# CookiePPP/cookietts

Hardware: AMD Instinct MI355X
Metric: audio samples/sec (22.05kHz) WaveGlow infer, 80×900 mel, 1/2/4/8 GPU; real-time factor (higher is better)
Workload: dtype f32; 1 GPU; WaveGlow full (12 flows, 512 WN ch, 8 groups, 8 layers) fp32 infer, batch 8 x (80x900) mel per GPU, sigma 0.6, random-init weights; batch_per_gpu=8, frames=900, parallelism=utterance-batch shard x1

## Files before the change

### cookietts_amd/_lib.py

```python
from __future__ import annotations

import ctypes as C
import os
import threading

import torch

from . import build as _build

_LOCK = threading.Lock()
_LIB = None


class WaveGlowConfig(C.Structure):
    _fields_ = [(n, C.c_int32) for n in (
        "n_mel_channels", "n_group", "n_flows", "n_early_every", "n_early_size",
        "win_length", "hop_length", "n_layers", "n_channels", "kernel_size", "cond_hidden", "speaker_embed_dim",
        "f32_gemm_mode")]


class StftConfig(C.Structure):
    _fields_ = [("filter_length", C.c_int32), ("hop_length", C.c_int32), ("win_length", C.c_int32),
                ("n_mel_channels", C.c_int32), ("clamp_val", C.c_float)]

# ... 269 lines not shown
                                           C.c_size_t, _FP]),
    "ctts_hifigan_packed_bf16x3_bytes": (C.c_size_t, [C.POINTER(HifiganConfig)]),
    "ctts_hifigan_pack_bf16x3": (C.c_int, [C.POINTER(HifiganConfig), _FP, C.c_size_t, _FP, _FP]),
    "ctts_hifigan_workspace_bf16x3_bytes": (C.c_size_t, [C.POINTER(HifiganConfig), C.c_int32, C.c_int32]),
    "ctts_hifigan_forward_bf16x3": (C.c_int, [C.POINTER(HifiganConfig), _FP, _FP, C.c_int32, _FP, C.c_int32, C.c_int32, _FP,
                                              C.c_size_t, _FP]),
    "ctts_replicate_halo_f32":(C.c_int, [_FP, C.c_int32, C.c_int32, C.c_int32, C.c_int32, C.c_int32, C.c_int32, _FP]),
    "ctts_embed_rows_f32": (C.c_int, [_FP, _FP, _FP, C.c_int32, C.c_int32, C.c_int32, C.c_int32, C.c_int32, C.c_int32,
                                      C.c_int32, _FP]),
    "ctts_scale_add_rows_f32": (C.c_int, [_FP, _FP, _FP, _FP, C.c_int32, C.c_int32, C.c_int32, C.c_int32, C.c_int32,
                                          _FP]),
    "ctts_deemphasis_f32": (C.c_int, [_FP, _FP, C.c_int32, C.c_int32, C.c_double, _FP]),
    "ctts_alignment_workspace_bytes": (C.c_size_t, [C.c_int32, C.c_int32, C.c_int32]),
    "ctts_alignment_metric_f32": (C.c_int, [_FP, _FP, _FP, C.c_int32, C.c_int32, C.c_int32, C.c_float, _FP, _FP,
                                            C.c_size_t, _FP]),
    "ctts_first_over_thresh_f32": (C.c_int, [_FP, C.c_int32, C.c_int32, C.c_float, _FP, _FP]),
    "ctts_taco_stop_state_bytes": (C.c_size_t, [C.c_int32]),
    "ctts_taco_stop_reset": (C.c_int, [_FP, C.c_int32, C.c_int32, _FP]),
    "ctts_taco_stop_rule_f32": (C.c_int, [_FP, C.c_int32, C.c_int32, C.c_int32, C.c_int32, C.c_float, C.c_int32, _FP, _FP]),
    "ctts_retry_state_bytes": (C.c_size_t, [C.POINTER(RetryConfig)]),
    "ctts_retry_state_layout": (C.c_int, [C.POINTER(RetryConfig), C.POINTER(C.c_size_t)]),
    "ctts_retry_reset": (C.c_int, [C.POINTER(RetryConfig), _FP, _FP]),
    "ctts_retry_update_f32": (C.c_int, [C.POINTER(RetryConfig), _FP, _FP, _FP, _FP, _FP, _FP, C.c_int32, C.c_int32, _FP, _FP,
                                        _FP]),
    "ctts_retry_vocoder_batch_f32": (C.c_int, [C.POINTER(RetryConfig), _FP, _FP, C.c_int32, C.c_float, _FP]),
    "ctts_pcm16_concat": (C.c_int, [_FP, C.c_int32, _FP, C.c_int32, C.c_int64, C.c_int32, C.c_int32, _FP, C.c_int64, _FP,
                                    _FP]),
    "ctts_affine_rows_f32": (C.c_int, [_FP, C.c_int32, C.c_int32, C.c_int32, C.c_int32, C.c_int32, C.c_int32, C.c_float,
                                       C.c_float, _FP]),
    "ctts_vol_unscale_f32": (C.c_int, [_FP, C.c_int64, _FP]),
    "ctts_resample_rows_f32": (C.c_int, [_FP, _FP] + [C.c_int32] * 9 + [C.c_float, _FP]),
    "ctts_interleave_phases_f32": (C.c_int, [_FP, _FP] + [C.c_int32] * 10 + [_FP]),
    "ctts_last_gemm_loop": (C.c_int, []),
    "ctts_tuning_reload": (C.c_int, []),
    "ctts_tuning_flags": (C.c_int, []),
    "ctts_profile_create": (C.c_int, [C.POINTER(C.c_void_p)]),
    "ctts_profile_bind": (C.c_int, [C.c_void_p]),
    "ctts_profile_collect": (C.c_int, [C.c_void_p, C.c_int32, C.POINTER(C.c_int64), C.POINTER(C.c_double)]),
    "ctts_profile_destroy": (C.c_int, [C.c_void_p]),
}

MODEL_GEMM_MODES = {None: 0, "default": 0, "f32": 1, "bf16x3": 2, "bf16x6": 3}
GEMM_MODES = {"f32": 1, "bf16x3": 2, "bf16x6": 3}


def model_gemm_mode(mode):
    try:
        return MODEL_GEMM_MODES[mode]
    except KeyError:
        raise ValueError(f"f32 GEMM mode {mode!r}: expected one of 'default', 'f32', 'bf16x3', 'bf16x6'") from None


def set_f32_gemm_mode(mode):
    if mode in (None, "default", "f32"):
        return "f32"
    raise RuntimeError(f"cookietts_amd.set_f32_gemm_mode({mode!r}): the process-wide default was removed; "
                       f"call model.set_f32_gemm_mode({mode!r}) on each model instead")


class Profile:

    def __init__(self):
        h = C.c_void_p()
        check(lib().ctts_profile_create(C.byref(h)), "ctts_profile_create")
        self._h = h

# ... 121 lines not shown
```

### cookietts_amd/csrc/waveglow_api.hip

```cpp
#include <mutex>
#include <vector>

#include "gemm_bf16.h"
#include "gemm_f32.h"
#include "tuning.h"
#include "waveglow_kernels.h"
#include "wn_winograd_layer.h"

namespace ctts {

static thread_local char g_err[512] = "";

void set_error(const char* fmt, ...) {
    va_list ap;
    va_start(ap, fmt);
    vsnprintf(g_err, sizeof(g_err), fmt, ap);
    va_end(ap);
}

namespace {

constexpr size_t ALIGN_F = 64;
inline size_t align_up(size_t v) { return (v + ALIGN_F - 1) / ALIGN_F * ALIGN_F; }
constexpr int A_TILE = GEMM_KC * GEMM_BM;
// ... 121 lines not shown

struct Geom { int L, ld, pad, ntiles; };

int make_geom(const Plan& p, int frames, Geom& g) {
    CTTS_CHECK_ARG(frames >= 1, "frames=%d", frames);
    const long long T = (long long)frames * p.c.hop_length;
    g.L = (int)(T / p.c.n_group);
    int maxd = 1 << (p.c.n_layers - 1);
    g.pad = round_up(maxd > 128 ? maxd : 128, 32);
    g.ntiles = (g.L + GEMM_BN - 1) / GEMM_BN;
    g.ld = round_up(g.L, 256) + 2 * g.pad;
    return CTTS_OK;
}

struct PairGeom { int d, Lp, ntiles; };
PairGeom pair_geom(const Geom& g, int layer) {
    const int d = 1 << layer;
    const int Lp = (g.L + 2 * d - 1) / (2 * d) * d;
    return {d, Lp, (Lp + GEMM_BN - 1) / GEMM_BN};
}
int pair_ld(const Plan& p, const Geom& g) {
    int nt = 0;
    for (int i = 0; i < p.c.n_layers; ++i) nt = std::max(nt, pair_geom(g, i).ntiles);
    return nt * GEMM_BN;
}
PairGeom quad_geom(const Geom& g, int layer) {
    const int d = 1 << layer;
    const int Lq = (g.L + 4 * d - 1) / (4 * d) * d;
    return {d, Lq, (Lq + 63) / 64};
}
int quad_ld(const Plan& p, const Geom& g) {
    int nt = 0;
    for (int i = 0; i < p.c.n_layers; ++i) nt = std::max(nt, quad_geom(g, i).ntiles);
    return nt * 64;
}
constexpr long long WINOGRAD_MIN_COLS = 28800;
bool winograd_engages(const Plan& p, const Geom& g) {
    const Tuning t = tuning();
    if (t.f32_no_winograd || gemm_split_level(p.c.f32_gemm_mode) != 0) return false;
    const long long min_cols = t.f32_winograd_min >= 0 ? t.f32_winograd_min : WINOGRAD_MIN_COLS;
    return (long long)g.L >= min_cols;
}

constexpr long long WINOGRAD_FUSED_MIN_COLS = 28800;
bool winograd_fused_engages(const Plan& p, const Geom& g) {
    const Tuning t = tuning();
    if (t.f32_winograd_no_fused || t.f32_winograd_plain || t.f32_no_glds || !wn_winograd_layer_supported(p.C, p.H)) return false;
    const long long min_cols = t.f32_winograd_fused_min >= 0 ? t.f32_winograd_fused_min : WINOGRAD_FUSED_MIN_COLS;
    return winograd_engages(p, g) && (long long)g.L >= min_cols;
}

constexpr long long WINOGRAD_F43_MIN_COLS = 28800;
bool winograd_f43_engages(const Plan& p, const Geom& g) {
    const Tuning t = tuning();
    if (t.f32_winograd_no_f43 || !wn_winograd_layer_f43_supported(p.C, p.H) || !gemm_f32_dma_staged(p.nch_rs + p.nch1h)) return false;
    const long long min_cols = t.f32_winograd_f43_min >= 0 ? t.f32_winograd_f43_min : WINOGRAD_F43_MIN_COLS;
    return winograd_fused_engages(p, g) && (long long)g.L >= min_cols;
}

struct Workspace {
    float *audio, *spect, *spk, *h_tmp, *h_all, *x, *act, *out;
    float* act_all;
    float* a16;
    float* skend;
    float *wgV, *wgT, *wgH;
    int ldp, ldq;
    size_t total;
// ... 96 lines not shown
        a.nseg = 2;
        a.seg[1] = {spk, (long long)p.c.n_flows * p.S * g.ld, p.S / GEMM_KC, 0, p.S, 0};
    }
    a.dst0 = h_tmp; a.dst0_bstride = hstride; a.acc0 = 0;
    a.dst1 = h_tmp; a.dst1_bstride = hstride; a.acc1 = 0;
    a.split = p.c.n_flows * GEMM_BM;
    a.M = p.c.n_flows * GEMM_BM;
    int rc = launch_gemm_f32(GEMM_EPI_SPLIT, a, s);
    if (rc) return rc;
    a.A = blob + p.cond1_A; a.bias = blob + p.cond1_b;
    a.nseg = 1; a.nch_total = p.nch1h;
    a.seg[0] = {h_tmp, hstride, p.nch1h, 0, GEMM_BM, 0};
    a.dst0 = h_all; a.dst1 = h_all;
    return launch_gemm_f32(GEMM_EPI_SPLIT, a, s);
}

struct WnFold { float* a16; float* skend; float* audio; float* wave; };
struct WnWinograd { float* V; float* T; float* Hc; int ldp; int ldq; };

int run_in_layer_winograd(const Plan& p, const Geom& g, const float* blob, int k, int i, const float* x, const float* h_all,
                          float* act, const WnWinograd& wg, int batch, hipStream_t s) {
    const auto& f = p.fl[k];
    const PairGeom pg = pair_geom(g, i);
    const int C = p.C, H = p.H, ldp = wg.ldp;
    const long long hstride = (long long)p.c.n_flows * H * g.ld;
    const size_t vplane = (size_t)batch * C * ldp, tplane = (size_t)batch * 2 * C * ldp, hplane = (size_t)batch * H * ldp;
    const bool lean = !tuning().f32_winograd_plain && gemm_f32_dma_staged(p.nch_rs + p.nch1h);
    const bool in_place = lean && pg.d % 4 == 0;
    const bool fused = lean && winograd_fused_engages(p, g);
    const float* h2 = h_all + (size_t)k * H * g.ld;
    if (fused && wg.ldq > 0 && winograd_f43_engages(p, g)) {
        const PairGeom qg = quad_geom(g, i);
        const int ldq = wg.ldq;
        int rc = launch_winograd_transform_quad(x, (long long)C * g.ld, h2, hstride, wg.V, wg.Hc, batch, C, H, qg.d, g.L, qg.Lp, g.ld, g.pad,
                                                ldq, qg.ntiles * 64, !in_place, s);
        if (rc) return rc;
        WnWinogradLayerArgs w{};
        w.form = WNWG_F43;
        w.A_T2 = blob + f.wq_U_A[0][i]; w.A_T3 = blob + f.wq_U_A[1][i]; w.A_T4 = blob + f.wq_U_A[2][i]; w.A_T5 = blob + f.wq_U_A[3][i];
        w.A_e = blob + f.wq_e_A[i]; w.A_o = blob + f.wq_o_A[i];
        w.bias = blob + f.in_b[i];
        w.V = wg.V; w.vplane = (long long)batch * C * ldq;
        w.Hc = wg.Hc; w.hplane = (long long)batch * H * ldq;
        w.h2 = h2; w.h_bstride = hstride;
        w.act = act; w.act_bstride = (long long)C * g.ld;
        w.C = C; w.H = H; w.batch = batch;
        w.ldp = ldq; w.Lp = qg.Lp; w.ntiles = qg.ntiles;
        w.d = qg.d; w.L = g.L; w.ld = g.ld; w.pad = g.pad;
        w.in_place = in_place;
        return launch_wn_winograd_layer(w, s);
    }
    int rc = launch_winograd_transform(x, (long long)C * g.ld, h2, hstride, wg.V, wg.Hc, batch, C, H, pg.d, g.L, pg.Lp, g.ld, g.pad,
                                       ldp, pg.ntiles * GEMM_BN, !in_place, lean, s);
    if (rc) return rc;
    if (fused) {
        WnWinogradLayerArgs w{};
        w.A_T2 = blob + f.wg_T2_A[i]; w.A_T3 = blob + f.wg_T3_A[i]; w.A_e = blob + f.wg_e_A[i]; w.A_o = blob + f.wg_o_A[i];
        w.bias = blob + f.in_b[i];
        w.V = wg.V; w.vplane = (long long)vplane;
        w.Hc = wg.Hc; w.hplane = (long long)hplane;
        w.h2 = h2; w.h_bstride = hstride;
        w.act = act; w.act_bstride = (long long)C * g.ld;
        w.C = C; w.H = H; w.batch = batch;
        w.ldp = ldp; w.Lp = pg.Lp; w.ntiles = pg.ntiles;
        w.d = pg.d; w.L = g.L; w.ld = g.ld; w.pad = g.pad;
        w.in_place = in_place;
        return launch_wn_winograd_layer(w, s);
    }
// ... 806 lines not shown
}

int ctts_waveglow_infer_spk_f32(const ctts_waveglow_config* cfg, const void* packed, const float* mel,
                                const float* z_scaled, const int64_t* speaker_ids, float* wave, int32_t batch,
                                int32_t frames, void* workspace, size_t workspace_bytes, void* stream) {
    Plan p; Geom g; Workspace w;
    int rc = make_plan(cfg, p); if (rc) return rc;
    rc = make_geom(p, frames, g); if (rc) return rc;
    CTTS_CHECK_ARG(packed && mel && z_scaled && wave && workspace && batch >= 1, "infer: bad argument");
    carve(p, g, batch, static_cast<float*>(workspace), w);
    if (w.total * sizeof(float) > workspace_bytes) {
        set_error("infer: workspace %zu bytes < required %zu", workspace_bytes, w.total * sizeof(float));
        return CTTS_E_WORKSPACE;
    }
    hipStream_t s = as_stream(stream);
    const float* blob = static_cast<const float*>(packed);
    CTTS_CHECK_HIP(hipMemcpyAsync(w.audio, z_scaled, (size_t)batch * p.c.n_group * g.L * sizeof(float),
                                  hipMemcpyDeviceToDevice, s));
    rc = launch_upsample_squeeze(mel, blob + p.up_w, p.up_mfma ? blob + p.up_wp : nullptr, blob + p.up_b, w.spect, batch, p.c.n_mel_channels, frames,
                                 p.c.win_length, p.c.hop_length, p.c.n_group, g.ld, g.pad, s);
    if (rc) return rc;
    rc = fill_speaker_rows(p, g, blob, speaker_ids, w.spk, batch, s);
    if (rc) return rc;
    rc = run_cond(p, g, blob, w.spect, w.spk, w.h_tmp, w.h_all, batch, s);
    if (rc) return rc;
    for (int k = p.c.n_flows - 1; k >= 0; --k) {
        rc = run_flow(p, g, blob, k, w, w.audio, w.h_all, k == 0 ? wave : nullptr, batch, s);
        if (rc) return rc;
    }
    return CTTS_OK;
}

int ctts_last_gemm_loop(void) { return last_gemm_loop(); }
int ctts_tuning_reload(void) { reload_tuning(); return CTTS_OK; }
int ctts_tuning_flags(void) {
    const Tuning t = tuning();
    return (t.f32_no_glds ? 1 : 0) | (t.no_xcd_pair ? 2 : 0) | (t.bf16_no_wide ? 8 : 0) | (t.bf16_no_pp ? 16 : 0) |
           (t.wf_no_fuse ? 128 : 0) | (t.taco_no_fuse ? 256 : 0) | (t.f32_no_small ? 512 : 0) | (t.f32_force_small ? 1024 : 0) |
           (t.f32_no_splitk ? 2048 : 0) | (t.wf_no_vec_interp ? 4096 : 0) | (t.f32_no_defer_skip ? 8192 : 0) |
           (t.wf_no_region_split ? 16384 : 0) | (t.wf_no_row_queue ? 32768 : 0) | (t.wf_row_queue_min >= 0 ? 65536 : 0) |
           (t.wf_inject_abort ? 131072 : 0) | (t.wf_queue_debug ? 262144 : 0) | (t.f32_no_round_split ? 524288 : 0) |
           (t.bf16_ps ? (1 << 20) : 0) | (t.bf16_no_ps ? (1 << 21) : 0) | (t.taco_poll_delay_set ? (1 << 23) : 0) |
           (t.taco_valu ? (1 << 24) : 0) | (t.up_no_mfma ? (1 << 25) : 0) | (t.f32_no_wn_fold ? (1 << 26) : 0) |
           (t.taco_bg_no_pipe ? (1 << 27) : 0) | (t.f32_no_winograd ? (1 << 28) : 0) | (t.f32_winograd_min >= 0 ? (1 << 29) : 0) |
           (t.f32_winograd_plain ? (1 << 30) : 0) | (t.f32_winograd_fused_min >= 0 ? 4 : 0) | (t.f32_winograd_no_fused ? 32 : 0) |
           (t.f32_winograd_f43_min >= 0 ? (1 << 6) : 0) | (t.f32_winograd_no_f43 ? (1 << 22) : 0) |
           (t.wf_fwd_rowwise ? (int)(1u << 31) : 0);
}

int ctts_profile_create(void** handle) {
    CTTS_CHECK_ARG(handle, "profile_create: NULL");
    *handle = new Prof();
    return CTTS_OK;
}

int ctts_profile_bind(void* handle) {
    t_prof = static_cast<Prof*>(handle);
    return CTTS_OK;
}

int ctts_profile_collect(void* handle, int32_t which, int64_t* launches, double* total_ms) {
    Prof* pr = static_cast<Prof*>(handle);
    CTTS_CHECK_ARG(pr && which >= 0 && which < CTTS_PROF_N && launches && total_ms, "profile_collect: bad argument");
    std::lock_guard<std::mutex> lk(pr->mu);
    double tot = 0.0;
    int64_t n = 0;
// ... 218 lines not shown
```

### cookietts_amd/csrc/wn_winograd_layer.h

```cpp
#pragma once

#include "common.h"
#include "gemm_f32.h"

namespace ctts {

constexpr int WNWG_MAX_CHUNKS = 320;
constexpr int WNWG_F23 = 0, WNWG_F43 = 1;

struct WnWinogradLayerArgs {
    const float *A_T2, *A_T3, *A_e, *A_o, *bias;
    const float *A_T4, *A_T5;
    const float* V; long long vplane;
    const float* Hc; long long hplane;
    const float* h2; long long h_bstride;
    float* act; long long act_bstride;
    int C, H, batch;
    int ldp, Lp, ntiles;
    int d, L, ld, pad;
    int in_place;
    int form;
    int kt, kt_total, b0, col0;
};

bool wn_winograd_layer_supported(int C, int H);
bool wn_winograd_layer_f43_supported(int C, int H);
int launch_wn_winograd_layer(const WnWinogradLayerArgs& a, hipStream_t stream);

}
```

### cookietts_amd/csrc/wn_winograd_layer.hip

```cpp
#include "wn_winograd_layer.h"
#include "tuning.h"

namespace ctts {

typedef float wg_f32x16 __attribute__((ext_vector_type(16)));

namespace {

__device__ __forceinline__ float wg_sigmoid(float u) {
    return __builtin_amdgcn_rcpf(1.0f + __builtin_amdgcn_exp2f(u * -1.4426950408889634f));
}
__device__ __forceinline__ float wg_tanh(float u) {
    return 1.0f - 2.0f * __builtin_amdgcn_rcpf(1.0f + __builtin_amdgcn_exp2f(u * 2.8853900817779268f));
}

}

template <int NT, int F43>
__global__ __launch_bounds__(256, 2) void wn_winograd_layer_f32_kernel(const WnWinogradLayerArgs a) {
    static_assert(!F43 || NT == 1, "the F(4,3) form runs on the 64-column shape");
    constexpr int NI = F43 ? 4 : 2;
    constexpr int BN = 64 * NT;
    constexpr int A_ST = GEMM_KC * 128;
    constexpr int STG = A_ST + GEMM_KC * BN;
    constexpr int TAB = 3 * STG;
    constexpr int BIAS = TAB + 4 * WNWG_MAX_CHUNKS;
    constexpr int UPR = BN / 4;
    constexpr int RPP = 64 / UPR;
    __shared__ __attribute__((aligned(16))) float lds[BIAS + 128];

    const int t = threadIdx.x;
    const int lane = t & 63;
    const int wave = __builtin_amdgcn_readfirstlane(t >> 6);
    const int wm = wave >> 1, wn = wave & 1;
    const int l31 = lane & 31, lhi = lane >> 5;

    const int ncb = a.C >> 6;
    const int jx = blockIdx.x >> 3;
    const int cb = jx % ncb;
    const int gt = (jx / ncb) * 8 + (blockIdx.x & 7);
    if (gt >= a.kt_total) return;
    const int b = a.b0 + gt / a.kt;
    const int n0 = a.col0 + (gt % a.kt) * BN;

    const int n1 = a.C / GEMM_KC, n2 = (a.C + a.H) / GEMM_KC, nh = a.H / GEMM_KC;
    const int c_e = NI * n1;
    int ps[NI + 1];
    ps[0] = c_e;
#pragma unroll
    for (int k = 0; k < NI; ++k) ps[k + 1] = ps[k] + (k == 0 || k == NI - 1 ? n2 : nh);
    const int nch = ps[NI];

    const int mb_t = (64 * cb) >> 8, loc_t = (64 * cb) & 255;
    const int mb_s = (a.C + 64 * cb) >> 8, loc_s = (a.C + 64 * cb) & 255;
    {
        uint4* tab = reinterpret_cast<uint4*>(lds + TAB);
        for (int c = t; c < nch; c += 256) {
// ... 33 lines not shown
#pragma unroll
        for (int j = 0; j < NT; ++j) {
            const int krow = (wave + 4 * j) * RPP + lane / UPR;
            offb[j] = (unsigned)(((size_t)krow * a.ldp + bcol) * 4);
#pragma unroll
            for (int k = 0; k < NI; ++k) offb_m[k][j] = 0;
            if (a.in_place) {
                const int q = n0 + bcol;
                const int te = (q / a.d) * (NI * a.d) + q % a.d;
                const int lim = (a.ld - a.pad - 4) & ~3;
#pragma unroll
                for (int k = 0; k < NI; ++k) offb_m[k][j] = (unsigned)(((size_t)krow * a.ld + a.pad + min(te + k * a.d, lim)) * 4);
            }
        }
    }
    int m_lo[NI];
#pragma unroll
    for (int k = 0; k < NI; ++k) m_lo[k] = a.in_place ? ps[k] + (k == 0 || k == NI - 1 ? n1 : 0) : 0x7fffffff;

    wg_f32x16 X[NI][2][NT];
#pragma unroll
    for (int k = 0; k < NI; ++k)
#pragma unroll
        for (int i = 0; i < 2; ++i)
#pragma unroll
            for (int j = 0; j < NT; ++j)
#pragma unroll
                for (int r = 0; r < 16; ++r) X[k][i][j][r] = 0.0f;
    __syncthreads();

    typedef __attribute__((address_space(3))) float* lds_fptr;
    typedef const __attribute__((address_space(1))) float* gfloat_ptr;
    typedef const __attribute__((address_space(1))) char* gbyte_ptr;
    const uint4* ctab = reinterpret_cast<const uint4*>(lds + TAB);
#define WNWG_ADDR(buf, c)                                                                                   \
    lds_fptr la_ = (lds_fptr)(lds + (buf) * STG + wave * 256);                                              \
    const uint4 e_ = ctab[c];                                                                               \
    const bool as_ = (c) < c_e;                                       \
    bool mk_[NI];                                                     \
    _Pragma("unroll") for (int k = 0; k < NI; ++k) mk_[k] = (c) >= m_lo[k] && (c) < ps[k + 1];
#define WNWG_BASES()                                                                                        \
    const gbyte_ptr ac_ = reinterpret_cast<gbyte_ptr>(                                                      \
        ((unsigned long long)(unsigned)__builtin_amdgcn_readfirstlane((int)e_.y) << 32) |                   \
        (unsigned)__builtin_amdgcn_readfirstlane((int)e_.x));                                               \
    const gbyte_ptr bp_ = reinterpret_cast<gbyte_ptr>(                                                      \
        ((unsigned long long)(unsigned)__builtin_amdgcn_readfirstlane((int)e_.w) << 32) |                   \
        (unsigned)__builtin_amdgcn_readfirstlane((int)e_.z));
#define WNWG_PIECE(p)                                                                                       \
    do {                                                                                                    \
        if constexpr ((p) < 2) {                                                                            \
            unsigned o_ = as_ ? offa_s[(p)] : offa_g[(p)];                                                  \
            asm volatile("" : "+v"(o_));                                                                    \
            __builtin_amdgcn_global_load_lds((gfloat_ptr)(ac_ + o_), la_ + 1024 * (p), 16, 0, 0);           \
        } else if constexpr ((p) < 2 + NT) {                                                                \
            unsigned o_ = offb[(p) - 2];                                                                    \
            _Pragma("unroll") for (int k = 0; k < NI; ++k) o_ = mk_[k] ? offb_m[k][(p) - 2] : o_;           \
            asm volatile("" : "+v"(o_));                                                                    \
            __builtin_amdgcn_global_load_lds((gfloat_ptr)(bp_ + o_), la_ + A_ST + 1024 * ((p) - 2), 16, 0, 0); \
        }                                                                                                   \
    } while (0)
#define WNWG_WAIT()                                                                                         \
    do {                                                                                                    \
        if constexpr (NT == 2) asm volatile("s_waitcnt vmcnt(4)" ::: "memory");                             \
        else asm volatile("s_waitcnt vmcnt(3)" ::: "memory");                                               \
    } while (0)

    {
        { WNWG_ADDR(0, 0) WNWG_BASES() WNWG_PIECE(0); WNWG_PIECE(1); WNWG_PIECE(2); WNWG_PIECE(3); }
        { WNWG_ADDR(1, 1) WNWG_BASES() WNWG_PIECE(0); WNWG_PIECE(1); WNWG_PIECE(2); WNWG_PIECE(3); }
        WNWG_WAIT();
        __builtin_amdgcn_s_barrier();
        __builtin_amdgcn_sched_barrier(0);
    }

    int cur = 0;
#define WNWG_READ_FRAGS(ks)                                                                                 \
    _Pragma("unroll") for (int mt = 0; mt < 2; ++mt) av[ks][mt] = As[(2 * (ks) + lhi) * 128 + mt * 64];     \
    _Pragma("unroll") for (int nt = 0; nt < NT; ++nt) bv[ks][nt] = Bs[(2 * (ks) + lhi) * BN + nt * 32];
#define WNWG_MFMA(Y, ks)                                                                                    \
    _Pragma("unroll") for (int mt = 0; mt < 2; ++mt)                                                        \
        _Pragma("unroll") for (int nt = 0; nt < NT; ++nt)                                                   \
            Y[mt][nt] = __builtin_amdgcn_mfma_f32_32x32x2f32(av[ks][mt], bv[ks][nt], Y[mt][nt], 0, 0, 0);
#define WNWG_REGION(Y, ks, p)                                                                               \
    __builtin_amdgcn_sched_barrier(0);                                                                      \
    if constexpr ((ks) + 1 < GEMM_KC / 2) { WNWG_READ_FRAGS((ks) + 1) }                                     \
    WNWG_MFMA(Y, ks)                                                                                        \
    WNWG_PIECE(p);
#define WNWG_CHUNK(Y)                                                                                       \
    {                                                                                                       \
        const float* As = lds + cur * STG + wm * 32 + l31;                                                  \
        const float* Bs = lds + cur * STG + A_ST + wn * (32 * NT) + l31;                                    \
        float av[GEMM_KC / 2][2], bv[GEMM_KC / 2][NT];                                                      \
        const int nb = cur >= 1 ? cur - 1 : 2;                \
        const int cn = ch + 2 < nch ? ch + 2 : nch - 1;                                                     \
        WNWG_ADDR(nb, cn)                                                                                   \
        WNWG_READ_FRAGS(0)                                                                                  \
        __builtin_amdgcn_sched_barrier(0);                                                                  \
        WNWG_BASES()                                                                                        \
        WNWG_REGION(Y, 0, 0) WNWG_REGION(Y, 1, 1) WNWG_REGION(Y, 2, 2) WNWG_REGION(Y, 3, 3)                 \
        WNWG_REGION(Y, 4, 4) WNWG_REGION(Y, 5, 4) WNWG_REGION(Y, 6, 4) WNWG_REGION(Y, 7, 4)                 \
        __builtin_amdgcn_sched_barrier(0);                                                                  \
        WNWG_WAIT();                                         \
        __builtin_amdgcn_s_barrier();                                                                       \
        __builtin_amdgcn_sched_barrier(0);                                                                  \
        cur = cur == 2 ? 0 : cur + 1;                                                                       \
    }

    float* dst = a.act + (size_t)b * a.act_bstride + (size_t)(cb * 64 + wm * 32) * a.ld + a.pad;
    const float* bias = lds + BIAS + wm * 32;
#define WNWG_GATE(Y, par)                                                                                   \
    _Pragma("unroll") for (int nt = 0; nt < NT; ++nt) {                                                     \
        const int n = n0 + wn * (32 * NT) + nt * 32 + l31;                                                  \
        const int ns = (n / a.d) * (NI * a.d) + n % a.d + (par) * a.d;                                      \
        if (n < a.Lp && ns < a.L) {                                                                         \
            _Pragma("unroll") for (int r = 0; r < 16; ++r) {                                                \
                const int row = (r & 3) + 8 * (r >> 2) + 4 * lhi;                                           \
                const float u0 = Y[0][nt][r] + bias[row];                                                   \
                const float u1 = Y[1][nt][r] + bias[64 + row];                                              \
                dst[(size_t)row * a.ld + ns] = wg_tanh(u0) * wg_sigmoid(u1);                                \
            }                                                                                               \
        }                                                                                                   \
    }

#define WNWG_RUN(k, end) for (; ch < (end); ++ch) WNWG_CHUNK(X[k])
#define WNWG_DRAIN()                                                                                        \
    asm volatile("s_waitcnt vmcnt(0)" ::: "memory");          \
    __builtin_amdgcn_s_barrier();
    int ch = 0;
    if constexpr (!F43) {
        WNWG_RUN(0, n1)
        WNWG_RUN(1, c_e)
#pragma unroll
        for (int i = 0; i < 2; ++i)
#pragma unroll
            for (int j = 0; j < NT; ++j)
#pragma unroll
                for (int r = 0; r < 16; ++r) {
                    const float s = X[0][i][j][r], dd = X[1][i][j][r];
                    X[0][i][j][r] = s + dd;
                    X[1][i][j][r] = s - dd;
                }
        WNWG_RUN(0, ps[1])
        WNWG_GATE(X[0], 0)
        WNWG_RUN(1, nch)
        WNWG_DRAIN()
        WNWG_GATE(X[1], 1)
    } else {
        WNWG_RUN(0, n1)
        WNWG_RUN(1, 2 * n1)
        WNWG_RUN(2, 3 * n1)
        WNWG_RUN(3, c_e)
#pragma unroll
        for (int i = 0; i < 2; ++i)
#pragma unroll
            for (int j = 0; j < NT; ++j)
#pragma unroll
                for (int r = 0; r < 16; ++r) {
                    const float p1 = X[0][i][j][r], p2 = X[1][i][j][r], p3 = X[2][i][j][r], p4 = X[3][i][j][r];
                    const float sa = p1 + p2, sb = p1 - p2, sc = p3 + p4, se = p3 - p4;
                    X[0][i][j][r] = sa + sc;
                    X[1][i][j][r] = sb + 2.0f * se;
                    X[2][i][j][r] = sa + 4.0f * sc;
                    X[3][i][j][r] = sb + 8.0f * se;
                }
#pragma unroll
        for (int k = 0; k < NI; ++k)
#pragma unroll
            for (int i = 0; i < 2; ++i) asm volatile("" : "+v"(X[k][i][0]));
        WNWG_RUN(0, ps[1])
        WNWG_GATE(X[0], 0)
        WNWG_RUN(1, ps[2])
        WNWG_GATE(X[1], 1)
        WNWG_RUN(2, ps[3])
        WNWG_GATE(X[2], 2)
        WNWG_RUN(3, nch)
        WNWG_DRAIN()
        WNWG_GATE(X[3], 3)
    }
#undef WNWG_DRAIN
#undef WNWG_RUN
#undef WNWG_GATE
#undef WNWG_CHUNK
#undef WNWG_REGION
#undef WNWG_MFMA
#undef WNWG_READ_FRAGS
#undef WNWG_WAIT
#undef WNWG_PIECE
#undef WNWG_BASES
#undef WNWG_ADDR
}

bool wn_winograd_layer_supported(int C, int H) {
    return C >= 128 && C % 128 == 0 && H > 0 && H % GEMM_KC == 0 && 2 * (C / GEMM_KC) + 2 * ((C + H) / GEMM_KC) <= WNWG_MAX_CHUNKS;
}

bool wn_winograd_layer_f43_supported(int C, int H) {
    return wn_winograd_layer_supported(C, H) && 4 * (C / GEMM_KC) + 2 * ((C + H) / GEMM_KC) + 2 * (H / GEMM_KC) <= WNWG_MAX_CHUNKS;
}

namespace {
template <int NT, int F43 = 0>
int launch_wnwg_shape(WnWinogradLayerArgs a, int kt, long long kt_total, hipStream_t stream) {
    a.kt = kt;
    a.kt_total = (int)kt_total;
    const long long blocks = 8ll * (a.C / 64) * ((kt_total + 7) / 8);
    CTTS_CHECK_ARG(blocks > 0 && blocks < (1ll << 31) && kt_total < (1ll << 31), "wn_winograd_layer: grid %lld", blocks);
    hipLaunchKernelGGL((wn_winograd_layer_f32_kernel<NT, F43>), dim3((unsigned)blocks), dim3(256), 0, stream, a);
    CTTS_CHECK_LAUNCH("wn_winograd_layer");
    return CTTS_OK;
}
}

int launch_wn_winograd_layer(const WnWinogradLayerArgs& a_in, hipStream_t stream) {
    WnWinogradLayerArgs a = a_in;
    CTTS_CHECK_ARG(wn_winograd_layer_supported(a.C, a.H), "wn_winograd_layer: C=%d H=%d", a.C, a.H);
    CTTS_CHECK_ARG(a.A_T2 && a.A_T3 && a.A_e && a.A_o && a.bias && a.V && a.act && a.batch >= 1, "wn_winograd_layer: operand not set");
    const bool f43 = a.form == WNWG_F43;
    const int tw = f43 ? 64 : 128;
    CTTS_CHECK_ARG(a.form == WNWG_F23 || (f43 && wn_winograd_layer_f43_supported(a.C, a.H) && a.A_T4 && a.A_T5), "wn_winograd_layer: form %d", a.form);
    CTTS_CHECK_ARG(a.d >= 1 && a.L >= 1 && a.Lp >= 1 && a.ntiles >= 1 && a.Lp <= a.ntiles * tw && a.ntiles * tw <= a.ldp && a.ldp % 4 == 0 &&
                       a.ld % 4 == 0 && a.pad >= 0 && a.pad % 4 == 0 && a.L + a.pad <= a.ld,
                   "wn_winograd_layer: geometry d=%d L=%d Lp=%d ntiles=%d ldp=%d ld=%d pad=%d", a.d, a.L, a.Lp, a.ntiles, a.ldp, a.ld, a.pad);
    CTTS_CHECK_ARG(a.in_place ? (a.h2 && a.d % 4 == 0 && a.ld - a.pad >= 4 && a.h_bstride % 4 == 0 && reinterpret_cast<uintptr_t>(a.h2) % 16 == 0)
                              : a.Hc != nullptr,
                   "wn_winograd_layer: cond rows (in_place=%d d=%d)", a.in_place, a.d);
    a.b0 = 0;
    a.col0 = 0;
    if (f43) return launch_wnwg_shape<1, 1>(a, a.ntiles, (long long)a.ntiles * a.batch, stream);
    const Tuning tn = tuning();
    const int ncb = a.C / 64;
    const long long slots = 2ll * wf_row_cus();
    const int kt_narrow = (a.Lp + 63) / 64;
    long long tiles = (long long)a.ntiles * a.batch;
    if (!tn.f32_no_small && (tn.f32_force_small || ncb * tiles < 2 * slots)) return launch_wnwg_shape<1>(a, kt_narrow, (long long)kt_narrow * a.batch, stream);
    if (!tn.f32_no_round_split && !tn.f32_no_small) {
        const long long rounds = ncb * tiles / slots;
        const long long rem_tiles = (ncb * tiles - rounds * slots + ncb - 1) / ncb;
        if (rounds >= 2 && rem_tiles > 0 && rem_tiles * ncb <= slots * 3 / 10 && rem_tiles < a.ntiles &&
            (long long)(a.ntiles - rem_tiles) * 128 < a.Lp) {
            WnWinogradLayerArgs r = a;
            r.b0 = a.batch - 1;
            r.col0 = (int)(a.ntiles - rem_tiles) * 128;
            const int kt = (a.Lp - r.col0 + 63) / 64;
            if (int rc = launch_wnwg_shape<1>(r, kt, kt, stream)) return rc;
            tiles -= rem_tiles;
        }
    }
    return launch_wnwg_shape<2>(a, a.ntiles, tiles, stream);
}

}
```

### include/cookietts_hip.h

```cpp
#ifndef COOKIETTS_HIP_H
#define COOKIETTS_HIP_H

#include <stddef.h>
#include <stdint.h>

#ifdef __cplusplus
extern "C" {
#endif

#define CTTS_OK 0
#define CTTS_E_ARG (-1)
#define CTTS_E_LAUNCH (-2)
#define CTTS_E_WORKSPACE (-3)
#define CTTS_E_ABORT (-4)

#define CTTS_ABI_VERSION 7

#define CTTS_GEMM_DEFAULT 0
#define CTTS_GEMM_F32 1
#define CTTS_GEMM_BF16X3 2
#define CTTS_GEMM_BF16X6 3
#define CTTS_N_SPEAKERS 512

int ctts_abi_version(void);
// ... 536 lines not shown
                            float gate_threshold, int32_t gate_delay, void* state, void* stream);

typedef struct ctts_retry_config {
    double diagonality_weighting, max_focus_weighting, min_focus_weighting, avg_focus_weighting;
    double target_score, absolutely_required_score;
    int32_t max_attempts, absolute_maximum_tries;
    int32_t n_texts, per_text;
    int32_t n_mel, t_cap, enc_cap;
} ctts_retry_config;

typedef struct ctts_retry_status {
    int32_t done;
    int32_t n_passes;
    double min_best_score;
    int32_t min_tries;
    int32_t n_without_winner;
    int32_t max_best_length;
    int32_t max_best_T;
} ctts_retry_status;

size_t ctts_retry_state_bytes(const ctts_retry_config* cfg);
#define CTTS_RETRY_SECTIONS 14
int ctts_retry_state_layout(const ctts_retry_config* cfg, size_t* offsets);
int ctts_retry_reset(const ctts_retry_config* cfg, void* state, void* stream);
int ctts_retry_update_f32(const ctts_retry_config* cfg, const float* mel, const float* gate, const float* alignments,
                          const double* metrics, const int32_t* output_lengths, const int32_t* text_lengths, int32_t T,
                          int32_t enc, double* detail, void* state, void* stream);
int ctts_retry_vocoder_batch_f32(const ctts_retry_config* cfg, const void* state, float* mel_out, int32_t t_out,
                                 float pad_value, void* stream);
int ctts_pcm16_concat(const void* audio, int32_t is_half, const int32_t* frames, int32_t batch, int64_t ld, int32_t hop,
                      int32_t silence_samples, int16_t* pcm, int64_t pcm_capacity, int64_t* offsets, void* stream);

int ctts_last_gemm_loop(void);

int ctts_tuning_reload(void);
int ctts_tuning_flags(void);

#define CTTS_PROF_WN_IN 0
#define CTTS_PROF_WN_RS 1
#define CTTS_PROF_WN_SKIP 2
#define CTTS_PROF_WN_IN0F 3
#define CTTS_PROF_WN_SKEND 4
#define CTTS_PROF_WN_RES_F 5
#define CTTS_PROF_N 6
int ctts_profile_create(void** handle);
int ctts_profile_bind(void* handle);
int ctts_profile_collect(void* handle, int32_t which, int64_t* launches, double* total_ms);
int ctts_profile_destroy(void* handle);

#ifdef __cplusplus
}
#endif
#endif
```

Before: 3.842 million samples/s.

## Deepen F(4,3) Winograd WN pipeline with two K chunks per stage and prefetched chunk table

The F(4,3) Winograd WN layer kernel gains a variant that stages two K chunks per pipeline stage and software-prefetches the per-chunk address table via explicit ds_read_b128. It also adds an optional 128-column wide shape, with quad ld padded to 128, behind the no_small tuning flag. By default, with H divisible by 2*KC, the 64-column KD=2 prefetch variant runs. The aim is to cut barrier and LDS table-read latency per chunk. In exchange it doubles the LDS stage size, which may reduce occupancy, and uses more registers for fragments. A debug query for the chosen F(4,3) width is added.

```diff
diff --git a/cookietts_amd/_lib.py b/cookietts_amd/_lib.py
--- a/cookietts_amd/_lib.py
+++ b/cookietts_amd/_lib.py
@@ -325,6 +325,7 @@
     "ctts_resample_rows_f32": (C.c_int, [_FP, _FP] + [C.c_int32] * 9 + [C.c_float, _FP]),
     "ctts_interleave_phases_f32": (C.c_int, [_FP, _FP] + [C.c_int32] * 10 + [_FP]),
     "ctts_last_gemm_loop": (C.c_int, []),
+    "ctts_last_winograd_f43_width": (C.c_int, []),
     "ctts_tuning_reload": (C.c_int, []),
     "ctts_tuning_flags": (C.c_int, []),
     "ctts_profile_create": (C.c_int, [C.POINTER(C.c_void_p)]),
diff --git a/cookietts_amd/csrc/waveglow_api.hip b/cookietts_amd/csrc/waveglow_api.hip
--- a/cookietts_amd/csrc/waveglow_api.hip
+++ b/cookietts_amd/csrc/waveglow_api.hip
@@ -177,7 +177,7 @@
 int quad_ld(const Plan& p, const Geom& g) {
     int nt = 0;
     for (int i = 0; i < p.c.n_layers; ++i) nt = std::max(nt, quad_geom(g, i).ntiles);
-    return nt * 64;
+    return round_up(nt * 64, 128);
 }
 constexpr long long WINOGRAD_MIN_COLS = 28800;
 bool winograd_engages(const Plan& p, const Geom& g) {
@@ -340,8 +340,9 @@
     if (fused && wg.ldq > 0 && winograd_f43_engages(p, g)) {
         const PairGeom qg = quad_geom(g, i);
         const int ldq = wg.ldq;
+        const int ncols = tuning().f32_no_small ? round_up(qg.ntiles * 64, 128) : qg.ntiles * 64;
         int rc = launch_winograd_transform_quad(x, (long long)C * g.ld, h2, hstride, wg.V, wg.Hc, batch, C, H, qg.d, g.L, qg.Lp, g.ld, g.pad,
-                                                ldq, qg.ntiles * 64, !in_place, s);
+                                                ldq, ncols, !in_place, s);
         if (rc) return rc;
         WnWinogradLayerArgs w{};
         w.form = WNWG_F43;
@@ -1214,6 +1215,7 @@
 }
 
 int ctts_last_gemm_loop(void) { return last_gemm_loop(); }
+int ctts_last_winograd_f43_width(void) { return last_wn_winograd_f43_width(); }
 int ctts_tuning_reload(void) { reload_tuning(); return CTTS_OK; }
 int ctts_tuning_flags(void) {
     const Tuning t = tuning();
diff --git a/cookietts_amd/csrc/wn_winograd_layer.h b/cookietts_amd/csrc/wn_winograd_layer.h
--- a/cookietts_amd/csrc/wn_winograd_layer.h
+++ b/cookietts_amd/csrc/wn_winograd_layer.h
@@ -26,5 +26,6 @@
 bool wn_winograd_layer_supported(int C, int H);
 bool wn_winograd_layer_f43_supported(int C, int H);
 int launch_wn_winograd_layer(const WnWinogradLayerArgs& a, hipStream_t stream);
+int last_wn_winograd_f43_width();
 
 }
diff --git a/cookietts_amd/csrc/wn_winograd_layer.hip b/cookietts_amd/csrc/wn_winograd_layer.hip
--- a/cookietts_amd/csrc/wn_winograd_layer.hip
+++ b/cookietts_amd/csrc/wn_winograd_layer.hip
@@ -4,6 +4,7 @@
 namespace ctts {
 
 typedef float wg_f32x16 __attribute__((ext_vector_type(16)));
+typedef unsigned wg_u32x4 __attribute__((ext_vector_type(4)));
 
 namespace {
 
@@ -16,13 +17,15 @@
 
 }
 
-template <int NT, int F43>
-__global__ __launch_bounds__(256, 2) void wn_winograd_layer_f32_kernel(const WnWinogradLayerArgs a) {
-    static_assert(!F43 || NT == 1, "the F(4,3) form runs on the 64-column shape");
+template <int NT, int F43, int KD, int TP>
+__global__ __launch_bounds__(256, (F43 && NT == 2) ? 1 : 2) void wn_winograd_layer_f32_kernel(const WnWinogradLayerArgs a) {
+    static_assert(KD == 1 || (KD == 2 && F43 && TP), "two chunks per stage: the F(4,3) form (its phases are whole stages, see the launcher)");
     constexpr int NI = F43 ? 4 : 2;
     constexpr int BN = 64 * NT;
     constexpr int A_ST = GEMM_KC * 128;
-    constexpr int STG = A_ST + GEMM_KC * BN;
+    constexpr int CST = A_ST + GEMM_KC * BN;
+    constexpr int STG = KD * CST;
+    constexpr int NP = 2 + NT;
     constexpr int TAB = 3 * STG;
     constexpr int BIAS = TAB + 4 * WNWG_MAX_CHUNKS;
     constexpr int UPR = BN / 4;
@@ -122,42 +125,66 @@
     typedef __attribute__((address_space(3))) float* lds_fptr;
     typedef const __attribute__((address_space(1))) float* gfloat_ptr;
     typedef const __attribute__((address_space(1))) char* gbyte_ptr;
-    const uint4* ctab = reinterpret_cast<const uint4*>(lds + TAB);
+    const wg_u32x4* ctab = reinterpret_cast<const wg_u32x4*>(lds + TAB);
+    wg_u32x4 tn_[KD];
+    const unsigned tab_lds = (unsigned)reinterpret_cast<uintptr_t>((lds_fptr)(lds + TAB));
+#define WNWG_TAB_ISSUE(c)                                                                                   \
+    _Pragma("unroll") for (int j = 0; j < KD; ++j) asm volatile("ds_read_b128 %0, %1" : "=v"(tn_[j]) : "v"(tab_lds + 16u * (unsigned)((c) + j)));
+#define WNWG_TAB_WAIT()                                                                                     \
+    do {                                                                                                    \
+        if constexpr (KD == 2) asm volatile("s_waitcnt lgkmcnt(0)" : "+v"(tn_[0]), "+v"(tn_[KD - 1]) : : "memory"); \
+        else asm volatile("s_waitcnt lgkmcnt(0)" : "+v"(tn_[0]) : : "memory");                              \
+    } while (0)
 #define WNWG_ADDR(buf, c)                                                                                   \
     lds_fptr la_ = (lds_fptr)(lds + (buf) * STG + wave * 256);                                              \
-    const uint4 e_ = ctab[c];                                                                               \
+    wg_u32x4 e_[KD];                                                                                        \
+    _Pragma("unroll") for (int j = 0; j < KD; ++j) {                                                        \
+        if constexpr (TP) e_[j] = tn_[j];                                                                   \
+        else e_[j] = ctab[(c) + j];                                                                         \
+    }                                                                                                       \
     const bool as_ = (c) < c_e;                                       \
     bool mk_[NI];                                                     \
     _Pragma("unroll") for (int k = 0; k < NI; ++k) mk_[k] = (c) >= m_lo[k] && (c) < ps[k + 1];
 #define WNWG_BASES()                                                                                        \
-    const gbyte_ptr ac_ = reinterpret_cast<gbyte_ptr>(                                                      \
-        ((unsigned long long)(unsigned)__builtin_amdgcn_readfirstlane((int)e_.y) << 32) |                   \
-        (unsigned)__builtin_amdgcn_readfirstlane((int)e_.x));                                               \
-    const gbyte_ptr bp_ = reinterpret_cast<gbyte_ptr>(                                                      \
-        ((unsigned long long)(unsigned)__builtin_amdgcn_readfirstlane((int)e_.w) << 32) |                   \
-        (unsigned)__builtin_amdgcn_readfirstlane((int)e_.z));
+    gbyte_ptr ac_[KD], bp_[KD];                                                                             \
+    _Pragma("unroll") for (int j = 0; j < KD; ++j) {                                                        \
+        ac_[j] = reinterpret_cast<gbyte_ptr>(                                                               \
+            ((unsigned long long)(unsigned)__builtin_amdgcn_readfirstlane((int)e_[j].y) << 32) |            \
+            (unsigned)__builtin_amdgcn_readfirstlane((int)e_[j].x));                                        \
+        bp_[j] = reinterpret_cast<gbyte_ptr>(                                                               \
+            ((unsigned long long)(unsigned)__builtin_amdgcn_readfirstlane((int)e_[j].w) << 32) |            \
+            (unsigned)__builtin_amdgcn_readfirstlane((int)e_[j].z));                                        \
+    }
 #define WNWG_PIECE(p)                                                                                       \
     do {                                                                                                    \
-        if constexpr ((p) < 2) {                                                                            \
-            unsigned o_ = as_ ? offa_s[(p)] : offa_g[(p)];                                                  \
-            asm volatile("" : "+v"(o_));                                                                    \
-            __builtin_amdgcn_global_load_lds((gfloat_ptr)(ac_ + o_), la_ + 1024 * (p), 16, 0, 0);           \
-        } else if constexpr ((p) < 2 + NT) {                                                                \
-            unsigned o_ = offb[(p) - 2];                                                                    \
-            _Pragma("unroll") for (int k = 0; k < NI; ++k) o_ = mk_[k] ? offb_m[k][(p) - 2] : o_;           \
-            asm volatile("" : "+v"(o_));                                                                    \
-            __builtin_amdgcn_global_load_lds((gfloat_ptr)(bp_ + o_), la_ + A_ST + 1024 * ((p) - 2), 16, 0, 0); \
+        if constexpr ((p) < KD * NP) {                                                                      \
+            constexpr int sj_ = (p) / NP, q_ = (p) % NP;                                                    \
+            if constexpr (q_ < 2) {                                                                         \
+                unsigned o_ = as_ ? offa_s[q_] : offa_g[q_];                                                \
+                asm volatile("" : "+v"(o_));                                                                \
+                __builtin_amdgcn_global_load_lds((gfloat_ptr)(ac_[sj_] + o_), la_ + sj_ * CST + 1024 * q_, 16, 0, 0); \
+            } else {                                                                                        \
+                unsigned o_ = offb[q_ - 2];                                                                 \
+                _Pragma("unroll") for (int k = 0; k < NI; ++k) o_ = mk_[k] ? offb_m[k][q_ - 2] : o_;        \
+                asm volatile("" : "+v"(o_));                                                                \
+                __builtin_amdgcn_global_load_lds((gfloat_ptr)(bp_[sj_] + o_), la_ + sj_ * CST + A_ST + 1024 * (q_ - 2), 16, 0, 0); \
+            }                                                                                               \
         }                                                                                                   \
     } while (0)
 #define WNWG_WAIT()                                                                                         \
     do {                                                                                                    \
-        if constexpr (NT == 2) asm volatile("s_waitcnt vmcnt(4)" ::: "memory");                             \
+        if constexpr (KD * NP == 8) asm volatile("s_waitcnt vmcnt(8)" ::: "memory");                        \
+        else if constexpr (KD * NP == 6) asm volatile("s_waitcnt vmcnt(6)" ::: "memory");                   \
+        else if constexpr (KD * NP == 4) asm volatile("s_waitcnt vmcnt(4)" ::: "memory");                   \
         else asm volatile("s_waitcnt vmcnt(3)" ::: "memory");                                               \
     } while (0)
 
     {
-        { WNWG_ADDR(0, 0) WNWG_BASES() WNWG_PIECE(0); WNWG_PIECE(1); WNWG_PIECE(2); WNWG_PIECE(3); }
-        { WNWG_ADDR(1, 1) WNWG_BASES() WNWG_PIECE(0); WNWG_PIECE(1); WNWG_PIECE(2); WNWG_PIECE(3); }
+        if constexpr (TP) { WNWG_TAB_ISSUE(0) WNWG_TAB_WAIT(); }
+        { WNWG_ADDR(0, 0) WNWG_BASES() WNWG_PIECE(0); WNWG_PIECE(1); WNWG_PIECE(2); WNWG_PIECE(3); WNWG_PIECE(4); WNWG_PIECE(5); WNWG_PIECE(6); WNWG_PIECE(7); }
+        if constexpr (TP) { WNWG_TAB_ISSUE(KD) WNWG_TAB_WAIT(); }
+        { WNWG_ADDR(1, KD) WNWG_BASES() WNWG_PIECE(0); WNWG_PIECE(1); WNWG_PIECE(2); WNWG_PIECE(3); WNWG_PIECE(4); WNWG_PIECE(5); WNWG_PIECE(6); WNWG_PIECE(7); }
+        if constexpr (TP) { WNWG_TAB_ISSUE(2 * KD < nch ? 2 * KD : nch - KD) WNWG_TAB_WAIT(); }
         WNWG_WAIT();
         __builtin_amdgcn_s_barrier();
         __builtin_amdgcn_sched_barrier(0);
@@ -176,7 +203,7 @@
     if constexpr ((ks) + 1 < GEMM_KC / 2) { WNWG_READ_FRAGS((ks) + 1) }                                     \
     WNWG_MFMA(Y, ks)                                                                                        \
     WNWG_PIECE(p);
-#define WNWG_CHUNK(Y)                                                                                       \
+#define WNWG_CHUNK1(Y)                                                                                      \
     {                                                                                                       \
         const float* As = lds + cur * STG + wm * 32 + l31;                                                  \
         const float* Bs = lds + cur * STG + A_ST + wn * (32 * NT) + l31;                                    \
@@ -188,12 +215,61 @@
         __builtin_amdgcn_sched_barrier(0);                                                                  \
         WNWG_BASES()                                                                                        \
         WNWG_REGION(Y, 0, 0) WNWG_REGION(Y, 1, 1) WNWG_REGION(Y, 2, 2) WNWG_REGION(Y, 3, 3)                 \
-        WNWG_REGION(Y, 4, 4) WNWG_REGION(Y, 5, 4) WNWG_REGION(Y, 6, 4) WNWG_REGION(Y, 7, 4)                 \
-        __builtin_amdgcn_sched_barrier(0);                                                                  \
+        WNWG_REGION(Y, 4, 4)                                                                                \
+        if constexpr (TP) { WNWG_TAB_ISSUE(ch + 3 < nch ? ch + 3 : nch - 1) }                               \
+        WNWG_REGION(Y, 5, 4) WNWG_REGION(Y, 6, 4) WNWG_REGION(Y, 7, 4)                                      \
+        __builtin_amdgcn_sched_barrier(0);                                                                  \
+        if constexpr (TP) WNWG_TAB_WAIT();                                                                  \
         WNWG_WAIT();                                         \
         __builtin_amdgcn_s_barrier();                                                                       \
         __builtin_amdgcn_sched_barrier(0);                                                                  \
         cur = cur == 2 ? 0 : cur + 1;                                                                       \
+    }
+    float fa[8 * KD][2], fb[8 * KD][NT];
+#define WNWG_RD(r, Ap, Bp)                                                                                  \
+    _Pragma("unroll") for (int mt = 0; mt < 2; ++mt) fa[r][mt] = (Ap)[((r) >> 3) * CST + (2 * ((r) & 7) + lhi) * 128 + mt * 64]; \
+    _Pragma("unroll") for (int nt = 0; nt < NT; ++nt) fb[r][nt] = (Bp)[((r) >> 3) * CST + (2 * ((r) & 7) + lhi) * BN + nt * 32];
+#define WNWG_MM(Y, r)                                                                                       \
+    _Pragma("unroll") for (int mt = 0; mt < 2; ++mt)                                                        \
+        _Pragma("unroll") for (int nt = 0; nt < NT; ++nt)                                                   \
+            Y[mt][nt] = __builtin_amdgcn_mfma_f32_32x32x2f32(fa[r][mt], fb[r][nt], Y[mt][nt], 0, 0, 0);
+#define WNWG_R2(Y, r)                                                                                       \
+    __builtin_amdgcn_sched_barrier(0);                                                                      \
+    WNWG_RD((r) + 1, As, Bs)                                                                                \
+    WNWG_MM(Y, r)                                                                                           \
+    WNWG_PIECE(r);
+#define WNWG_CHUNK2(Y)                                                                                      \
+    {                                                                                                       \
+        const float* As = lds + cur * STG + wm * 32 + l31;                                                  \
+        const float* Bs = lds + cur * STG + A_ST + wn * (32 * NT) + l31;                                    \
+        const int nx = cur == 2 ? 0 : cur + 1;                                                              \
+        const float* An = lds + nx * STG + wm * 32 + l31;                                                   \
+        const float* Bn = lds + nx * STG + A_ST + wn * (32 * NT) + l31;                                     \
+        const int nb = cur >= 1 ? cur - 1 : 2;                      \
+        const int cn = ch + 2 * KD < nch ? ch + 2 * KD : nch - KD;                                          \
+        WNWG_ADDR(nb, cn)                                                                                   \
+        __builtin_amdgcn_sched_barrier(0);                                                                  \
+        WNWG_BASES()                                                                                        \
+        WNWG_R2(Y, 0) WNWG_R2(Y, 1) WNWG_R2(Y, 2) WNWG_R2(Y, 3) WNWG_R2(Y, 4) WNWG_R2(Y, 5) WNWG_R2(Y, 6) WNWG_R2(Y, 7)   \
+        WNWG_R2(Y, 8) WNWG_R2(Y, 9)                                                                         \
+        WNWG_TAB_ISSUE(ch + 3 * KD < nch ? ch + 3 * KD : nch - KD)                                          \
+        WNWG_R2(Y, 10) WNWG_R2(Y, 11) WNWG_R2(Y, 12) WNWG_R2(Y, 13) WNWG_R2(Y, 14)                          \
+        __builtin_amdgcn_sched_barrier(0);                                                                  \
+        WNWG_TAB_WAIT();                                                \
+        WNWG_WAIT();                                         \
+        __builtin_amdgcn_s_barrier();                                                                       \
+        __builtin_amdgcn_sched_barrier(0);                                                                  \
+        WNWG_RD(0, An, Bn)                                                                                  \
+        WNWG_MM(Y, 15)                                                                                      \
+        __builtin_amdgcn_sched_barrier(0);                                                                  \
+        cur = nx;                                                                                           \
+    }
+#define WNWG_CHUNK(Y)                                                                                       \
+    if constexpr (KD == 1) WNWG_CHUNK1(Y) else WNWG_CHUNK2(Y)
+    if constexpr (KD == 2) {
+        const float* As = lds + wm * 32 + l31;
+        const float* Bs = lds + A_ST + wn * (32 * NT) + l31;
+        WNWG_RD(0, As, Bs)
     }
 
     float* dst = a.act + (size_t)b * a.act_bstride + (size_t)(cb * 64 + wm * 32) * a.ld + a.pad;
@@ -212,7 +288,7 @@
         }                                                                                                   \
     }
 
-#define WNWG_RUN(k, end) for (; ch < (end); ++ch) WNWG_CHUNK(X[k])
+#define WNWG_RUN(k, end) for (; ch < (end); ch += KD) WNWG_CHUNK(X[k])
 #define WNWG_DRAIN()                                                                                        \
     asm volatile("s_waitcnt vmcnt(0)" ::: "memory");          \
     __builtin_amdgcn_s_barrier();
@@ -246,17 +322,24 @@
             for (int j = 0; j < NT; ++j)
 #pragma unroll
                 for (int r = 0; r < 16; ++r) {
+                    if constexpr (NT == 2)
+                        if (r == 0) asm volatile("" : "+a"(X[0][i][j]), "+a"(X[1][i][j]), "+a"(X[2][i][j]), "+a"(X[3][i][j]));
                     const float p1 = X[0][i][j][r], p2 = X[1][i][j][r], p3 = X[2][i][j][r], p4 = X[3][i][j][r];
                     const float sa = p1 + p2, sb = p1 - p2, sc = p3 + p4, se = p3 - p4;
                     X[0][i][j][r] = sa + sc;
                     X[1][i][j][r] = sb + 2.0f * se;
                     X[2][i][j][r] = sa + 4.0f * sc;
                     X[3][i][j][r] = sb + 8.0f * se;
+                    if constexpr (NT == 2)
+                        if (r == 15) asm volatile("" : "+a"(X[0][i][j]), "+a"(X[1][i][j]), "+a"(X[2][i][j]), "+a"(X[3][i][j]));
                 }
 #pragma unroll
         for (int k = 0; k < NI; ++k)
 #pragma unroll
-            for (int i = 0; i < 2; ++i) asm volatile("" : "+v"(X[k][i][0]));
+            for (int i = 0; i < 2; ++i) {
+                if constexpr (NT == 2) { asm volatile("" : "+a"(X[k][i][0])); asm volatile("" : "+a"(X[k][i][1])); }
+                else asm volatile("" : "+v"(X[k][i][0]));
+            }
         WNWG_RUN(0, ps[1])
         WNWG_GATE(X[0], 0)
         WNWG_RUN(1, ps[2])
@@ -271,12 +354,19 @@
 #undef WNWG_RUN
 #undef WNWG_GATE
 #undef WNWG_CHUNK
+#undef WNWG_CHUNK2
+#undef WNWG_R2
+#undef WNWG_MM
+#undef WNWG_RD
+#undef WNWG_CHUNK1
 #undef WNWG_REGION
 #undef WNWG_MFMA
 #undef WNWG_READ_FRAGS
 #undef WNWG_WAIT
 #undef WNWG_PIECE
 #undef WNWG_BASES
+#undef WNWG_TAB_WAIT
+#undef WNWG_TAB_ISSUE
 #undef WNWG_ADDR
 }
 
@@ -289,17 +379,22 @@
 }
 
 namespace {
-template <int NT, int F43 = 0>
+thread_local int t_last_f43_width = 0;
+
+template <int NT, int F43, int KD, int TP>
 int launch_wnwg_shape(WnWinogradLayerArgs a, int kt, long long kt_total, hipStream_t stream) {
     a.kt = kt;
     a.kt_total = (int)kt_total;
     const long long blocks = 8ll * (a.C / 64) * ((kt_total + 7) / 8);
     CTTS_CHECK_ARG(blocks > 0 && blocks < (1ll << 31) && kt_total < (1ll << 31), "wn_winograd_layer: grid %lld", blocks);
-    hipLaunchKernelGGL((wn_winograd_layer_f32_kernel<NT, F43>), dim3((unsigned)blocks), dim3(256), 0, stream, a);
+    hipLaunchKernelGGL((wn_winograd_layer_f32_kernel<NT, F43, KD, TP>), dim3((unsigned)blocks), dim3(256), 0, stream, a);
     CTTS_CHECK_LAUNCH("wn_winograd_layer");
     return CTTS_OK;
 }
-}
+
+}
+
+int last_wn_winograd_f43_width() { return t_last_f43_width; }
 
 int launch_wn_winograd_layer(const WnWinogradLayerArgs& a_in, hipStream_t stream) {
     WnWinogradLayerArgs a = a_in;
@@ -316,13 +411,24 @@
                    "wn_winograd_layer: cond rows (in_place=%d d=%d)", a.in_place, a.d);
     a.b0 = 0;
     a.col0 = 0;
-    if (f43) return launch_wnwg_shape<1, 1>(a, a.ntiles, (long long)a.ntiles * a.batch, stream);
     const Tuning tn = tuning();
+    if (f43) {
+        const bool kd2 = a.H % (2 * GEMM_KC) == 0;
+        if (tn.f32_no_small && kd2) {
+            const int wt = (a.ntiles + 1) / 2;
+            CTTS_CHECK_ARG((long long)wt * 128 <= a.ldp, "wn_winograd_layer: %d tiles of 128 quad columns beyond ldp=%d", wt, a.ldp);
+            t_last_f43_width = 128;
+            return launch_wnwg_shape<2, 1, 2, 1>(a, wt, (long long)wt * a.batch, stream);
+        }
+        t_last_f43_width = 64;
+        if (tn.f32_force_small || !kd2) return launch_wnwg_shape<1, 1, 1, 0>(a, a.ntiles, (long long)a.ntiles * a.batch, stream);
+        return launch_wnwg_shape<1, 1, 2, 1>(a, a.ntiles, (long long)a.ntiles * a.batch, stream);
+    }
     const int ncb = a.C / 64;
     const long long slots = 2ll * wf_row_cus();
     const int kt_narrow = (a.Lp + 63) / 64;
     long long tiles = (long long)a.ntiles * a.batch;
-    if (!tn.f32_no_small && (tn.f32_force_small || ncb * tiles < 2 * slots)) return launch_wnwg_shape<1>(a, kt_narrow, (long long)kt_narrow * a.batch, stream);
+    if (!tn.f32_no_small && (tn.f32_force_small || ncb * tiles < 2 * slots)) return launch_wnwg_shape<1, 0, 1, 0>(a, kt_narrow, (long long)kt_narrow * a.batch, stream);
     if (!tn.f32_no_round_split && !tn.f32_no_small) {
         const long long rounds = ncb * tiles / slots;
         const long long rem_tiles = (ncb * tiles - rounds * slots + ncb - 1) / ncb;
@@ -332,11 +438,11 @@
             r.b0 = a.batch - 1;
             r.col0 = (int)(a.ntiles - rem_tiles) * 128;
             const int kt = (a.Lp - r.col0 + 63) / 64;
-            if (int rc = launch_wnwg_shape<1>(r, kt, kt, stream)) return rc;
+            if (int rc = launch_wnwg_shape<1, 0, 1, 0>(r, kt, kt, stream)) return rc;
             tiles -= rem_tiles;
         }
     }
-    return launch_wnwg_shape<2>(a, a.ntiles, tiles, stream);
-}
-
-}
+    return launch_wnwg_shape<2, 0, 1, 0>(a, a.ntiles, tiles, stream);
+}
+
+}
diff --git a/include/cookietts_hip.h b/include/cookietts_hip.h
--- a/include/cookietts_hip.h
+++ b/include/cookietts_hip.h
@@ -592,6 +592,7 @@
                       int32_t silence_samples, int16_t* pcm, int64_t pcm_capacity, int64_t* offsets, void* stream);
 
 int ctts_last_gemm_loop(void);
+int ctts_last_winograd_f43_width(void);
 
 int ctts_tuning_reload(void);
 int ctts_tuning_flags(void);
```

Result: faster. 3.982 million samples/s (median of 6 runs) (+3.7%).
